# Gumo-A/hnsw_rs

Hardware: AMD Instinct MI355X
Metric: queries/sec at recall@10>=0.99, 1M x 100d L2 (higher is better)
Workload: dtype f32

## Files before the change

hnsw_rs_amd/csrc/capi.cpp:

```cpp

#include <hip/hip_runtime.h>

#include <linux/futex.h>
#include <sys/resource.h>
#include <sys/syscall.h>
#include <unistd.h>

#include <algorithm>
#include <atomic>
#include <chrono>
#include <climits>
#include <condition_variable>
#include <cstdio>
#include <cstdlib>
#include <cstring>
#include <memory>
#include <mutex>
#include <new>
#include <string>
#include <thread>
#include <vector>

#include "deleted.h"
#include "device_build.h"
#include "device_index.h"
#include "hip_util.h"
#include "host_index.h"
#include "search_filtered.h"

using hx::DevBuf;
using hx::set_error;

struct SearchScratch {
    void *dev = nullptr, *pin = nullptr;
    size_t dev_cap = 0, pin_cap = 0;
    hipStream_t stream = nullptr;
    int device = -1;
    ~SearchScratch() {
        if (dev) (void)hipFree(dev);
        if (pin) (void)hipHostFree(pin);
        if (stream) (void)hipStreamDestroy(stream);
    }
};

struct SpinLock {
    std::atomic<uint32_t> v{0};
    void lock() {
        for (int spins = 0; spins < 128; spins++) {
            uint32_t exp = 0;
            if (v.load(std::memory_order_relaxed) == 0 && v.compare_exchange_weak(exp, 1, std::memory_order_acquire)) return;
#if defined(__x86_64__)
            __builtin_ia32_pause();
#endif
        }
        while (v.exchange(2, std::memory_order_acquire) != 0)
            (void)syscall(SYS_futex, reinterpret_cast<uint32_t *>(&v), FUTEX_WAIT_PRIVATE, 2, nullptr, nullptr, 0);
    }
    void unlock() {
        if (v.exchange(0, std::memory_order_release) == 2)
            (void)syscall(SYS_futex, reinterpret_cast<uint32_t *>(&v), FUTEX_WAKE_PRIVATE, 1, nullptr, nullptr, 0);
    }
};

struct CoBatch {
    SearchScratch s;
    size_t p_q = 0, p_out = 0;
    std::atomic<uint32_t> cap{0}, n{0}, ef{0}, dim{0};
    static constexpr uint64_t COUNT = 0xFFFFull, CLOSED = 1ull << 16, GEN = 1ull << 32;
    std::atomic<uint64_t> word{CLOSED};
    std::atomic<uint32_t> filed{0};
    struct Req {
        uint32_t *ids, *count;
    };
    std::vector<Req> reqs;
    struct alignas(64) Word {
        std::atomic<uint32_t> v{0};
    };
    static constexpr uint32_t WORDS = 16;
    Word done[WORDS];
    std::atomic<uint32_t> readers{0};
    int rc = HNSW_OK;
    std::string err;
    std::vector<int32_t> status;
};
struct Coalescer {
    std::atomic<CoBatch *> fast{nullptr};
    SpinLock mu;
    std::condition_variable_any cv;
    std::vector<CoBatch *> open;
    std::vector<std::unique_ptr<CoBatch>> all;
    std::vector<CoBatch *> idle;
    uint32_t in_flight = 0;
    std::atomic<uint32_t> last_size{1};
    std::atomic<int64_t> window_us{30};
    uint32_t depth = 3, cap = 1024;
    std::atomic<uint64_t> n_batches{0}, n_queries{0}, max_batch{0};
    std::atomic<uint64_t> ns_window{0}, ns_turn{0}, ns_gpu{0}, ns_handout{0};
};

struct hnsw_index {
    std::unique_ptr<hx::HostIndex> host;
    hx::DeviceIndex dev;
    int device = -1;
    int gpu_build = 0;
    uint32_t build_batch_max = 8192, build_batch_div = 8;
    bool incomplete_build = false;
    bool cosine = false;
    std::mutex mu;
    std::mutex pool_mu;
    std::vector<std::unique_ptr<SearchScratch>> pool;
    Coalescer co;
    std::atomic<uint64_t> n_uploads{0}, n_point_patches{0}, n_patch_fallbacks{0};
    int64_t filter_exact_max = 65536;
    std::atomic<uint64_t> n_filt_graph{0}, n_filt_exact{0}, n_filt_overflow{0};
    hx::DeletedSet del;
    std::atomic<uint64_t> n_del_graph{0}, n_del_exact{0}, n_del_overflow{0};
    hx::BuildStats build;
};

namespace {

hx::BuildTarget build_target(hnsw_index *h) {
    return {*h->host, h->dev, h->device, {h->build_batch_max, h->build_batch_div}, h->build};
}

inline bool is_replica(const hnsw_index *h) { return h->dev.replica; }
inline uint64_t index_len(const hnsw_index *h) { return is_replica(h) ? h->dev.view.n_points : h->host->len(); }
int reject_replica(const hnsw_index *h, const char *what) {
    if (!is_replica(h)) return HNSW_OK;
    set_error("%s: this handle is a device-only replica (hnsw_snapshot_adopt); it holds no host copy of the index", what);
    return HNSW_ERR_ARG;
}

int cosine_rows(const hnsw_index *h, const float *&rows, uint64_t n, std::vector<float> &keep, uint32_t nb_threads = 1) {
    if (!h->cosine || !rows) return HNSW_OK;
    const uint32_t d = h->host->dim;
    keep.resize((size_t)n * d);
    std::atomic<uint64_t> bad{UINT64_MAX};
    auto work = [&](uint64_t lo, uint64_t hi) {
        for (uint64_t i = lo; i < hi; i++) {
            const float *x = rows + i * d;
            float s = 0.0f;
            for (uint32_t e = 0; e < d; e++) {
                const float t = x[e] * x[e];
                s += t;
            }
            const float nrm = sqrtf(s);
            if (!(nrm > 0.0f) || !std::isfinite(nrm)) {
                uint64_t cur = bad.load();
                while (i < cur && !bad.compare_exchange_weak(cur, i)) {
                }
                return;
            }
            float *y = &keep[(size_t)i * d];
            for (uint32_t e = 0; e < d; e++) y[e] = x[e] / nrm;
        }
    };
    const unsigned nt = (unsigned)std::min<uint64_t>(std::max(1u, nb_threads), std::max<uint64_t>(1, n / 4096));
    if (nt <= 1) {
        work(0, n);
    } else {
        std::vector<std::thread> th;
        for (unsigned t = 0; t < nt; t++) th.emplace_back(work, n * t / nt, n * (t + 1) / nt);
        for (auto &t : th) t.join();
    }
    if (bad.load() != UINT64_MAX) {
        set_error("row %llu has no direction (zero, NaN, or a norm outside f32's range): the cosine metric cannot place it",
                  (unsigned long long)bad.load());
        return HNSW_ERR_NAN_INPUT;
    }
    rows = keep.data();
    return HNSW_OK;
}
int cosine_queries(const hnsw_index *h, void *d_Q, uint64_t nq, hipStream_t stream) {
    if (!h->cosine) return HNSW_OK;
    return hx::launch_normalise_rows(static_cast<float *>(d_Q), nq, h->dev.view.dim, stream);
}

struct DeviceQueries {
    const float *q = nullptr;
    void *tmp = nullptr;
    hipStream_t st = nullptr;
    int prepare(const hnsw_index *h, const float *d_Q, uint64_t nq, hipStream_t stream) {
        q = d_Q;
        st = stream;
        if (!h->cosine) return HNSW_OK;
        const size_t bytes = (size_t)nq * h->dev.view.dim * 4;
        HIP_TRY(hipMallocAsync(&tmp, bytes, stream));
        HIP_TRY(hipMemcpyAsync(tmp, d_Q, bytes, hipMemcpyDeviceToDevice, stream));
        q = static_cast<const float *>(tmp);
        return hx::launch_normalise_rows(static_cast<float *>(tmp), nq, h->dev.view.dim, stream);
    }
    ~DeviceQueries() {
        if (tmp) (void)hipFreeAsync(tmp, st);
    }
};

int ensure_uploaded(hnsw_index *h) {
    std::lock_guard<std::mutex> g(h->mu);
    if (is_replica(h) && !h->dev.valid) {
        set_error("replica snapshot not committed (hnsw_snapshot_commit)");
        return HNSW_ERR_ARG;
    }
    if (!h->dev.current(*h->host)) {
        int rc = h->dev.upload(*h->host, h->device);
        if (rc != HNSW_OK) return rc;
        h->device = h->dev.device;
        h->n_uploads.fetch_add(1, std::memory_order_relaxed);
        hipMemPool_t pool = nullptr;
        if (hipDeviceGetDefaultMemPool(&pool, h->dev.device) == hipSuccess && pool != nullptr) {
            uint64_t keep = 1ull << 30;
            (void)hipMemPoolSetAttribute(pool, hipMemPoolAttrReleaseThreshold, &keep);
        }
        (void)hipGetLastError();
    }
    hipError_t e = hipSetDevice(h->dev.device);
    if (e != hipSuccess) {
        set_error("hipSetDevice(%d): %s", h->dev.device, hipGetErrorString(e));
        return HNSW_ERR_HIP;
    }
    return HNSW_OK;
}

int check_search_args(const hnsw_index *h, uint32_t ef) {
    if (!h) {
        set_error("null handle");
        return HNSW_ERR_ARG;
    }
    if (h->incomplete_build) {
        set_error("an on-device build on this handle failed half way; the index is incomplete, discard it");
        return HNSW_ERR_ARG;
    }
    if (index_len(h) == 0) {
        set_error("index is empty");
        return HNSW_ERR_EMPTY;
    }
    if (ef > (1u << 26)) {
        set_error("ef = %u is above 2^26", ef);
        return HNSW_ERR_ARG;
    }
    return HNSW_OK;
}

hx::SearchArgs ann_args(const hx::DevView &v, const float *dQ, uint32_t n, uint32_t ef,
                        uint32_t *ids, float *dists, uint32_t *counts, hnsw_query_stats *stats) {
    hx::SearchArgs a{};
    a.Q = dQ;
    a.qsel = nullptr;
    a.entries = nullptr;
    a.n_entry = 1;
    a.layer_hi = (int32_t)v.nb_layers - 1;
    a.layer_lo = 0;
    a.ef_upper = 1;
    a.ef_bottom = ef;
    a.n = n;
    a.out_ids = ids;
    a.out_dists = dists;
    a.out_counts = counts;
    a.out_stats = stats;
    return a;
}

struct ScratchLease {
    hnsw_index *h;
    std::unique_ptr<SearchScratch> s;
    explicit ScratchLease(hnsw_index *hh) : h(hh) {
        std::lock_guard<std::mutex> g(h->pool_mu);
        if (!h->pool.empty()) {
            s = std::move(h->pool.back());
            h->pool.pop_back();
        }
    }
    ~ScratchLease() {
        if (!s) return;
        std::lock_guard<std::mutex> g(h->pool_mu);
        if (h->pool.size() < 16) h->pool.push_back(std::move(s));
    }
    int prepare(int device, size_t dev_bytes, size_t pin_bytes) {
        if (s && s->device != device) s.reset();
        if (!s) {
            s.reset(new SearchScratch());
            s->device = device;
            HIP_TRY(hipStreamCreateWithFlags(&s->stream, hipStreamNonBlocking));
        }
        if (s->dev_cap < dev_bytes) {
            if (s->dev) (void)hipFree(s->dev);
            s->dev = nullptr;
            s->dev_cap = 0;
            const size_t cap = dev_bytes + dev_bytes / 4 + 4096;
            HIP_TRY(hipMalloc(&s->dev, cap));
            s->dev_cap = cap;
        }
        if (s->pin_cap < pin_bytes) {
            if (s->pin) (void)hipHostFree(s->pin);
            s->pin = nullptr;
            s->pin_cap = 0;
            const size_t cap = pin_bytes + pin_bytes / 4 + 4096;
            HIP_TRY(hipHostMalloc(&s->pin, cap, hipHostMallocDefault));
            s->pin_cap = cap;
        }
        return HNSW_OK;
    }
};

inline size_t align256(size_t x) { return (x + 255) & ~(size_t)255; }

struct HostSearchPlan {
    size_t o_q, o_sel, o_ent, o_out, dev_bytes;
    size_t r_ids, r_dists, r_counts, r_stats, out_bytes;
    size_t p_q, p_out, pin_bytes;
};
HostSearchPlan plan_host_search(uint64_t nq, uint32_t d, uint32_t n, uint32_t n_entry) {
    HostSearchPlan p{};
    p.o_q = 0;
    p.o_sel = p.o_q + align256(nq * d * 4);
    p.o_ent = p.o_sel + align256(nq * 4);
    p.o_out = p.o_ent + align256((size_t)n_entry * 4);
    p.r_ids = 0;
    p.r_dists = p.r_ids + align256(nq * n * 4);
    p.r_counts = p.r_dists + align256(nq * n * 4);
    p.r_stats = p.r_counts + align256(nq * 4);
    p.out_bytes = p.r_stats + align256(nq * sizeof(hnsw_query_stats));
    p.dev_bytes = p.o_out + p.out_bytes;
    p.p_q = 0;
    p.p_out = align256(nq * d * 4);
    p.pin_bytes = p.p_out + p.out_bytes;
    return p;
}

int query_status_error(uint64_t i, int32_t status) {
    switch (status) {
        case HNSW_OK:
            break;
        case HNSW_ERR_NAN_INPUT:
            set_error("query %llu: NaN in the query or in a distance", (unsigned long long)i);
            break;
        case HNSW_ERR_NODE_NOT_IN_GRAPH:
            set_error("Error in search_layer: node not in Graph (query %llu)", (unsigned long long)i);
            break;
        case HNSW_ERR_OVERFLOW:
            set_error("query %llu: visited table exhausted at its largest size", (unsigned long long)i);
            break;
        default:
            set_error("query %llu failed with status %d", (unsigned long long)i, status);
    }
    return status;
}

int search_staged(hnsw_index *h, SearchScratch &s, const HostSearchPlan &p, hx::SearchArgs a_host, uint64_t nq,
                  const uint32_t *entries, const float *Q_user) {
    const hx::DevView &v = h->dev.view;
    unsigned char *dv = static_cast<unsigned char *>(s.dev), *hv = static_cast<unsigned char *>(s.pin);
    int rc;
    static const bool zc_allowed = !(getenv("HNSW_MI355X_ZERO_COPY") && atoi(getenv("HNSW_MI355X_ZERO_COPY")) == 0);
    static const uint64_t zc_max = getenv("HNSW_MI355X_ZERO_COPY_MAX") ? strtoull(getenv("HNSW_MI355X_ZERO_COPY_MAX"), nullptr, 0) : 512;
    const bool zc = zc_allowed && !Q_user && !h->cosine && nq <= zc_max;
    hx::SearchArgs a = a_host;
    unsigned char *ob = zc ? hv + p.p_out : dv + p.o_out;
    if (zc) {
        a.Q = reinterpret_cast<const float *>(hv + p.p_q);
    } else {
        HIP_TRY(hipMemcpyAsync(dv + p.o_q, Q_user ? (const void *)Q_user : (const void *)(hv + p.p_q), nq * v.dim * 4,
                               hipMemcpyHostToDevice, s.stream));
        if ((rc = cosine_queries(h, dv + p.o_q, nq, s.stream))) return rc;
        a.Q = reinterpret_cast<const float *>(dv + p.o_q);
    }
    a.out_ids = reinterpret_cast<uint32_t *>(ob + p.r_ids);
    a.out_dists = reinterpret_cast<float *>(ob + p.r_dists);
    a.out_counts = reinterpret_cast<uint32_t *>(ob + p.r_counts);
    a.out_stats = reinterpret_cast<hnsw_query_stats *>(ob + p.r_stats);
    if (entries) {
        HIP_TRY(hipMemcpyAsync(dv + p.o_ent, entries, (size_t)a.n_entry * 4, hipMemcpyHostToDevice, s.stream));
        a.entries = reinterpret_cast<const uint32_t *>(dv + p.o_ent);
    }
    const hnsw_query_stats *st = reinterpret_cast<const hnsw_query_stats *>(hv + p.p_out + p.r_stats);
    uint32_t ef_max = std::max(a.ef_bottom, a.ef_upper);
    uint32_t slots = hx::default_slots_log2(ef_max, v.S0);
    uint64_t nrun = nq;
    std::vector<uint32_t> sel;
    while (true) {
        rc = hx::launch_search(v, a, (uint32_t)nrun, slots, s.stream);
        if (rc != HNSW_OK) return rc;
        if (!zc) HIP_TRY(hipMemcpyAsync(hv + p.p_out, dv + p.o_out, p.out_bytes, hipMemcpyDeviceToHost, s.stream));
        HIP_TRY(hipStreamSynchronize(s.stream));
        sel.clear();
        for (uint64_t i = 0; i < nq; i++)
            if (st[i].status == HNSW_ERR_OVERFLOW) sel.push_back((uint32_t)i);
        if (sel.empty() || slots >= hx::max_slots_log2(ef_max)) break;
        slots++;
        HIP_TRY(hipMemcpyAsync(dv + p.o_sel, sel.data(), sel.size() * 4, hipMemcpyHostToDevice, s.stream));
        HIP_TRY(hipStreamSynchronize(s.stream));
        a.qsel = reinterpret_cast<const uint32_t *>(dv + p.o_sel);
        nrun = sel.size();
    }
    return HNSW_OK;
}

int search_host(hnsw_index *h, hx::SearchArgs a_host, const float *Q, uint64_t nq, uint32_t *ids,
                float *dists, uint32_t *counts, hnsw_query_stats *stats, const uint32_t *entries) {
    int rc = ensure_uploaded(h);
    if (rc != HNSW_OK) return rc;
    const hx::DevView &v = h->dev.view;
    const uint32_t n = a_host.n, d = v.dim;
    const HostSearchPlan p = plan_host_search(nq, d, n, entries ? a_host.n_entry : 0);
    const bool stage_q = nq * (size_t)d * 4 <= (8u << 20);
    ScratchLease lease(h);
    if ((rc = lease.prepare(h->dev.device, p.dev_bytes, stage_q ? p.pin_bytes : p.out_bytes))) return rc;
    SearchScratch &s = *lease.s;
    HostSearchPlan pp = p;
    if (!stage_q) pp.p_out = 0;
    unsigned char *hv = static_cast<unsigned char *>(s.pin);
    if (stage_q) memcpy(hv + pp.p_q, Q, nq * (size_t)d * 4);
    if ((rc = search_staged(h, s, pp, a_host, nq, entries, stage_q ? nullptr : Q))) return rc;
    const unsigned char *ob = hv + pp.p_out;
    const hnsw_query_stats *st = reinterpret_cast<const hnsw_query_stats *>(ob + pp.r_stats);
    memcpy(ids, ob + pp.r_ids, nq * n * 4);
    if (dists) memcpy(dists, ob + pp.r_dists, nq * n * 4);
    if (counts) memcpy(counts, ob + pp.r_counts, nq * 4);
    if (stats) memcpy(stats, st, nq * sizeof(hnsw_query_stats));
    for (uint64_t i = 0; i < nq; i++)
        if (st[i].status != HNSW_OK) return query_status_error(i, st[i].status);
    return HNSW_OK;
}


struct PathCounters {
    std::atomic<uint64_t> *graph, *exact, *overflow;
};
const uint64_t kNoWords = 0;

PathCounters filt_counters(hnsw_index *h) { return {&h->n_filt_graph, &h->n_filt_exact, &h->n_filt_overflow}; }
PathCounters del_counters(hnsw_index *h) { return {&h->n_del_graph, &h->n_del_exact, &h->n_del_overflow}; }

int sync_deleted(hnsw_index *h) {
    if (h->del.count == 0) return HNSW_OK;
    std::lock_guard<std::mutex> g(h->mu);
    if (h->del.d_words && h->del.d_device == h->dev.device && h->del.dirty.empty()) return HNSW_OK;
    ScratchLease lease(h);
    int rc = lease.prepare(h->dev.device, 0, 0);
    if (rc != HNSW_OK) return rc;
    return h->del.sync(h->dev.device, lease.s->stream);
}

uint64_t count_admissible(const hnsw_index *h, const uint64_t *allow, uint64_t bits, std::vector<uint32_t> &wbase) {
    const uint64_t n_words = (bits + 63) / 64, n_wblk = (n_words + 63) / 64;
    const std::vector<uint64_t> &deny = h->del.words;
    const bool denies = h->del.count > 0;
    wbase.assign(std::max<uint64_t>(1, n_wblk), 0);
    uint64_t A = 0;
    for (uint64_t w = 0; w < n_words; w++) {
        if (w % 64 == 0) wbase[w / 64] = (uint32_t)A;
        uint64_t x = allow ? allow[w] : ~0ull;
        if (w == n_words - 1 && bits % 64) x &= (1ull << (bits % 64)) - 1;
        if (denies && w < deny.size()) x &= ~deny[w];
        A += (uint64_t)__builtin_popcountll(x);
    }
    return A;
}

int filtered_exact(const hx::DevView &v, const hx::FilterArgs &a, uint64_t nsel, const uint32_t *d_sel, uint64_t n_words,
                   const uint32_t *d_wb, uint32_t *d_ids, uint64_t A, uint32_t chunk, uint32_t nseg, void *part,
                   void *pst, hipStream_t stream) {
    int r = hx::launch_filter_compact(a, n_words, d_wb, d_ids, stream);
    for (uint64_t c = 0; r == HNSW_OK && c < nsel; c += chunk) {
        hx::FilterArgs ac = a;
        if (d_sel) {
            ac.qsel = d_sel + c;
        } else {
            ac.qsel = nullptr;
            ac.Q += c * v.dim;
            ac.out_ids += c * a.n;
            ac.out_dists += c * a.n;
            ac.out_counts += c;
            ac.out_stats += c;
        }
        r = hx::launch_filtered_exact(v, ac, (uint32_t)std::min<uint64_t>(chunk, nsel - c), d_ids, (uint32_t)A, nseg,
                                      static_cast<unsigned long long *>(part), static_cast<int32_t *>(pst), stream);
    }
    return r;
}

int search_filtered(hnsw_index *h, const float *Q, uint64_t nq, uint32_t n, uint32_t ef, const uint64_t *allow,
                    uint64_t allow_bits, bool exact_only, uint32_t *ids, float *dists, uint32_t *counts,
                    hnsw_query_stats *stats, uint8_t *paths, const PathCounters *ctr) {
    int rc = check_search_args(h, ef);
    if (rc != HNSW_OK) return rc;
    if (nq == 0) return HNSW_OK;
    if (!Q || !ids || nq > 0x7FFFFFFFull || n > HX_FILT_MAX_N) {
        set_error("filtered search: needs queries, an id buffer, a mask when allow_bits > 0 and n <= %d",
                  HX_FILT_MAX_N);
        return HNSW_ERR_ARG;
    }
    if (n == 0) {
        if (counts) memset(counts, 0, nq * 4);
        return HNSW_OK;
    }
    const uint32_t efp = std::max(std::max(ef, n), 1u);
    const uint64_t bits = std::min<uint64_t>(allow_bits, index_len(h));
    const uint64_t n_words = (bits + 63) / 64;
    std::vector<uint32_t> wbase;
    const uint64_t A = count_admissible(h, allow, bits, wbase);
    const bool exact_all = exact_only || (int64_t)A <= h->filter_exact_max;
    if (!exact_all && efp > HX_FILT_MAX_EF) {
        set_error("filtered search: ef' = max(ef, n) = %u is above the graph path's maximum of %d", efp, HX_FILT_MAX_EF);
        return HNSW_ERR_ARG;
    }
    if ((rc = ensure_uploaded(h)) || (rc = sync_deleted(h))) return rc;
    const hx::DevView &v = h->dev.view;
    const uint32_t d = v.dim;
    const uint32_t chunk = (uint32_t)std::min<uint64_t>(nq, 65535);
    const uint32_t nseg = hx::filt_exact_segments(A, chunk);
    const size_t o_q = 0, o_mask = o_q + align256(nq * d * 4), o_wb = o_mask + align256(allow ? n_words * 8 : 0),
                 o_ids = o_wb + align256(wbase.size() * 4), o_sel = o_ids + align256(A * 4),
                 o_part = o_sel + align256(nq * 4), o_pst = o_part + align256((size_t)chunk * nseg * n * 8),
                 o_out = o_pst + align256((size_t)chunk * nseg * 4);
    const size_t r_ids = 0, r_dists = align256(nq * n * 4), r_counts = r_dists + align256(nq * n * 4),
                 r_stats = r_counts + align256(nq * 4), out_bytes = r_stats + align256(nq * sizeof(hnsw_query_stats));
    ScratchLease lease(h);
    if ((rc = lease.prepare(h->dev.device, o_out + out_bytes, out_bytes))) return rc;
    SearchScratch &s = *lease.s;
    unsigned char *dv = static_cast<unsigned char *>(s.dev), *hv = static_cast<unsigned char *>(s.pin);
    HIP_TRY(hipMemcpyAsync(dv + o_q, Q, nq * d * 4, hipMemcpyHostToDevice, s.stream));
    if ((rc = cosine_queries(h, dv + o_q, nq, s.stream))) return rc;
    if (n_words) {
        if (allow) HIP_TRY(hipMemcpyAsync(dv + o_mask, allow, n_words * 8, hipMemcpyHostToDevice, s.stream));
        HIP_TRY(hipMemcpyAsync(dv + o_wb, wbase.data(), wbase.size() * 4, hipMemcpyHostToDevice, s.stream));
    }
    hx::FilterArgs a{};
    a.Q = reinterpret_cast<const float *>(dv + o_q);
    a.allow = allow ? reinterpret_cast<const uint64_t *>(dv + o_mask) : nullptr;
    a.allow_bits = bits;
    a.deny = h->del.count ? h->del.d_words : nullptr;
    a.deny_bits = h->del.count ? h->del.deny_bits() : 0;
    a.n = n;
    a.ef = efp;
    a.out_ids = reinterpret_cast<uint32_t *>(dv + o_out + r_ids);
    a.out_dists = reinterpret_cast<float *>(dv + o_out + r_dists);
    a.out_counts = reinterpret_cast<uint32_t *>(dv + o_out + r_counts);
    a.out_stats = reinterpret_cast<hnsw_query_stats *>(dv + o_out + r_stats);
    uint32_t *d_sel = reinterpret_cast<uint32_t *>(dv + o_sel);
    auto exact = [&](uint64_t nsel, bool selected) -> int {
        return filtered_exact(v, a, nsel, selected ? d_sel : nullptr, n_words,
                              reinterpret_cast<const uint32_t *>(dv + o_wb), reinterpret_cast<uint32_t *>(dv + o_ids), A,
                              chunk, nseg, dv + o_part, dv + o_pst, s.stream);
    };
    const hnsw_query_stats *st = reinterpret_cast<const hnsw_query_stats *>(hv + r_stats);
    std::vector<uint8_t> path(nq, exact_all ? 1 : 0);
    if (exact_all) {
        if ((rc = exact(nq, false))) return rc;
        HIP_TRY(hipMemcpyAsync(hv, dv + o_out, out_bytes, hipMemcpyDeviceToHost, s.stream));
        HIP_TRY(hipStreamSynchronize(s.stream));
    } else {
        uint32_t slots = hx::filt_first_slots_log2(v, efp);
        const uint32_t max_slots = hx::filt_max_slots_log2(v);
        uint64_t nrun = nq;
        std::vector<uint32_t> sel;
        while (true) {
            if ((rc = hx::launch_filtered_graph(v, a, (uint32_t)nrun, slots, s.stream))) return rc;
            HIP_TRY(hipMemcpyAsync(hv, dv + o_out, out_bytes, hipMemcpyDeviceToHost, s.stream));
            HIP_TRY(hipStreamSynchronize(s.stream));
            sel.clear();
            for (uint64_t i = 0; i < nq; i++)
                if (st[i].status == HNSW_ERR_OVERFLOW) sel.push_back((uint32_t)i);
            if (sel.empty()) break;
            HIP_TRY(hipMemcpyAsync(d_sel, sel.data(), sel.size() * 4, hipMemcpyHostToDevice, s.stream));
            if (slots >= max_slots) {
                for (uint32_t i : sel) path[i] = 2;
                if ((rc = exact(sel.size(), true))) return rc;
                HIP_TRY(hipMemcpyAsync(hv, dv + o_out, out_bytes, hipMemcpyDeviceToHost, s.stream));
                HIP_TRY(hipStreamSynchronize(s.stream));
                break;
            }
            HIP_TRY(hipStreamSynchronize(s.stream));
            slots++;
            a.qsel = d_sel;
            nrun = sel.size();
        }
    }
    uint64_t n2 = 0;
    for (uint64_t i = 0; i < nq; i++) n2 += path[i] == 2;
    if (ctr) {
        if (exact_all)
            ctr->exact->fetch_add(nq, std::memory_order_relaxed);
        else
            ctr->graph->fetch_add(nq - n2, std::memory_order_relaxed);
        ctr->overflow->fetch_add(n2, std::memory_order_relaxed);
    }
    memcpy(ids, hv + r_ids, nq * n * 4);
    if (dists) memcpy(dists, hv + r_dists, nq * n * 4);
    if (counts) memcpy(counts, hv + r_counts, nq * 4);
    memcpy(stats, st, nq * sizeof(hnsw_query_stats));
    if (paths) memcpy(paths, path.data(), nq);
    return HNSW_OK;
}

int search_filtered_checked(hnsw_index *h, const float *Q, uint64_t nq, uint32_t n, uint32_t ef, const uint64_t *allow,
                            uint64_t allow_bits, bool exact_only, uint32_t *ids, float *dists, uint32_t *counts,
                            hnsw_query_stats *stats, uint8_t *paths, const PathCounters *ctr) {
    std::vector<hnsw_query_stats> local;
    if (!stats) {
        local.resize(nq);
        stats = local.data();
    }
    int rc = search_filtered(h, Q, nq, n, ef, allow, allow_bits, exact_only, ids, dists, counts, stats, paths, ctr);
    if (rc != HNSW_OK || n == 0) return rc;
    for (uint64_t i = 0; i < nq; i++)
        if (stats[i].status != HNSW_OK) return query_status_error(i, stats[i].status);
    return HNSW_OK;
}

int search_device_deleted(hnsw_index *h, const float *d_Q, uint64_t nq, uint32_t n, uint32_t ef, uint32_t *d_ids,
                          float *d_dists, uint32_t *d_counts, hnsw_query_stats *d_stats, hipStream_t stream, bool finish) {
    const uint32_t efp = std::max(std::max(ef, n), 1u);
    if (n > HX_FILT_MAX_N || efp > HX_FILT_MAX_EF) {
        set_error("search with deleted ids: needs n <= %d and ef' = max(ef, n) <= %d", HX_FILT_MAX_N, HX_FILT_MAX_EF);
        return HNSW_ERR_ARG;
    }
    int rc;
    if ((rc = ensure_uploaded(h)) || (rc = sync_deleted(h))) return rc;
    const hx::DevView &v = h->dev.view;
    DeviceQueries dq;
    if ((rc = dq.prepare(h, d_Q, nq, stream))) return rc;
    struct Tmp {
        void *p = nullptr;
        hipStream_t st = nullptr;
        ~Tmp() {
            if (p) (void)hipFreeAsync(p, st);
        }
    } t_dists, t_counts;
    if (!d_dists) {
        HIP_TRY(hipMallocAsync(&t_dists.p, nq * n * 4, stream));
        t_dists.st = stream;
        d_dists = static_cast<float *>(t_dists.p);
    }
    if (!d_counts) {
        HIP_TRY(hipMallocAsync(&t_counts.p, nq * 4, stream));
        t_counts.st = stream;
        d_counts = static_cast<uint32_t *>(t_counts.p);
    }
    hx::FilterArgs a{};
    a.Q = dq.q;
    a.allow = nullptr;
    a.allow_bits = index_len(h);
    a.deny = h->del.d_words;
    a.deny_bits = h->del.deny_bits();
    a.n = n;
    a.ef = efp;
    a.out_ids = d_ids;
    a.out_dists = d_dists;
    a.out_counts = d_counts;
    a.out_stats = d_stats;
    uint32_t slots = hx::filt_first_slots_log2(v, efp);
    if (!finish) return hx::launch_filtered_graph(v, a, (uint32_t)nq, slots, stream);

    const uint32_t max_slots = hx::filt_max_slots_log2(v);
    const size_t st_bytes = nq * sizeof(hnsw_query_stats);
    ScratchLease lease(h);
    if ((rc = lease.prepare(h->dev.device, align256(nq * 4), st_bytes))) return rc;
    hnsw_query_stats *st = static_cast<hnsw_query_stats *>(lease.s->pin);
    uint32_t *d_sel = static_cast<uint32_t *>(lease.s->dev);
    std::vector<uint32_t> sel;
    uint64_t n2 = 0;
    while (true) {
        HIP_TRY(hipMemcpyAsync(st, d_stats, st_bytes, hipMemcpyDeviceToHost, stream));
        HIP_TRY(hipStreamSynchronize(stream));
        sel.clear();
        for (uint64_t i = 0; i < nq; i++)
            if (st[i].status == HNSW_ERR_OVERFLOW) sel.push_back((uint32_t)i);
        if (sel.empty()) break;
        if (slots >= max_slots) {
            n2 = sel.size();
            std::vector<uint32_t> wbase;
            const uint64_t bits = a.allow_bits, n_words = (bits + 63) / 64;
            const uint64_t A = count_admissible(h, nullptr, bits, wbase);
            const uint32_t chunk = (uint32_t)std::min<uint64_t>(n2, 65535);
            const uint32_t nseg = hx::filt_exact_segments(A, chunk);
            const size_t o_sel = 0, o_wb = align256(n2 * 4), o_ids = o_wb + align256(wbase.size() * 4),
                         o_part = o_ids + align256(A * 4), o_pst = o_part + align256((size_t)chunk * nseg * n * 8),
                         bytes = o_pst + align256((size_t)chunk * nseg * 4);
            if ((rc = lease.prepare(h->dev.device, bytes, st_bytes))) return rc;
            unsigned char *dv = static_cast<unsigned char *>(lease.s->dev);
            st = static_cast<hnsw_query_stats *>(lease.s->pin);
            HIP_TRY(hipMemcpyAsync(dv + o_sel, sel.data(), n2 * 4, hipMemcpyHostToDevice, stream));
            HIP_TRY(hipMemcpyAsync(dv + o_wb, wbase.data(), wbase.size() * 4, hipMemcpyHostToDevice, stream));
            if ((rc = filtered_exact(v, a, n2, reinterpret_cast<const uint32_t *>(dv + o_sel), n_words,
                                     reinterpret_cast<const uint32_t *>(dv + o_wb), reinterpret_cast<uint32_t *>(dv + o_ids),
// ... 1376 lines not shown
```

Before: 6.065 million.

## Write search outputs directly to pinned host memory and pre-create pool streams

Search results (ids, dists, counts, stats) are now always written by the kernel straight into pinned host memory, even on the non-zero-copy path. This removes the device output buffer and the device-to-host copy after each launch. The first lease also creates several scratch streams up front so later concurrent searches do not pay stream creation cost. In exchange, large batches now write their outputs over the host interconnect, which may be slower than device writes followed by one bulk copy.

After: 6.044 million (median of 2 runs). About the same (-0.4%).

```diff
diff --git a/hnsw_rs_amd/csrc/capi.cpp b/hnsw_rs_amd/csrc/capi.cpp
--- a/hnsw_rs_amd/csrc/capi.cpp
+++ b/hnsw_rs_amd/csrc/capi.cpp
@@ -109,6 +109,7 @@
     std::mutex mu;
     std::mutex pool_mu;
     std::vector<std::unique_ptr<SearchScratch>> pool;
+    bool pool_primed = false;
     Coalescer co;
     std::atomic<uint64_t> n_uploads{0}, n_point_patches{0}, n_patch_fallbacks{0};
     int64_t filter_exact_max = 65536;
@@ -261,14 +262,19 @@
     return a;
 }
 
+constexpr unsigned kPoolStreamsUpFront = 4;
+
 struct ScratchLease {
     hnsw_index *h;
     std::unique_ptr<SearchScratch> s;
+    bool first = false;
     explicit ScratchLease(hnsw_index *hh) : h(hh) {
         std::lock_guard<std::mutex> g(h->pool_mu);
         if (!h->pool.empty()) {
             s = std::move(h->pool.back());
             h->pool.pop_back();
+        } else if (!h->pool_primed) {
+            h->pool_primed = first = true;
         }
     }
     ~ScratchLease() {
@@ -276,12 +282,24 @@
         std::lock_guard<std::mutex> g(h->pool_mu);
         if (h->pool.size() < 16) h->pool.push_back(std::move(s));
     }
+    static int make(int device, std::unique_ptr<SearchScratch> &out) {
+        out.reset(new SearchScratch());
+        out->device = device;
+        HIP_TRY(hipStreamCreateWithFlags(&out->stream, hipStreamNonBlocking));
+        HIP_TRY(hipStreamSynchronize(out->stream));
+        return HNSW_OK;
+    }
     int prepare(int device, size_t dev_bytes, size_t pin_bytes) {
         if (s && s->device != device) s.reset();
         if (!s) {
-            s.reset(new SearchScratch());
-            s->device = device;
-            HIP_TRY(hipStreamCreateWithFlags(&s->stream, hipStreamNonBlocking));
+            int rc = make(device, s);
+            if (rc != HNSW_OK) return rc;
+            for (unsigned i = 1; first && i < kPoolStreamsUpFront; i++) {
+                std::unique_ptr<SearchScratch> more;
+                if ((rc = make(device, more))) return rc;
+                std::lock_guard<std::mutex> g(h->pool_mu);
+                h->pool.insert(h->pool.begin(), std::move(more));
+            }
         }
         if (s->dev_cap < dev_bytes) {
             if (s->dev) (void)hipFree(s->dev);
@@ -306,7 +324,7 @@
 inline size_t align256(size_t x) { return (x + 255) & ~(size_t)255; }
 
 struct HostSearchPlan {
-    size_t o_q, o_sel, o_ent, o_out, dev_bytes;
+    size_t o_q, o_sel, o_ent, dev_bytes;
     size_t r_ids, r_dists, r_counts, r_stats, out_bytes;
     size_t p_q, p_out, pin_bytes;
 };
@@ -315,13 +333,12 @@
     p.o_q = 0;
     p.o_sel = p.o_q + align256(nq * d * 4);
     p.o_ent = p.o_sel + align256(nq * 4);
-    p.o_out = p.o_ent + align256((size_t)n_entry * 4);
     p.r_ids = 0;
     p.r_dists = p.r_ids + align256(nq * n * 4);
     p.r_counts = p.r_dists + align256(nq * n * 4);
     p.r_stats = p.r_counts + align256(nq * 4);
     p.out_bytes = p.r_stats + align256(nq * sizeof(hnsw_query_stats));
-    p.dev_bytes = p.o_out + p.out_bytes;
+    p.dev_bytes = p.o_ent + align256((size_t)n_entry * 4);
     p.p_q = 0;
     p.p_out = align256(nq * d * 4);
     p.pin_bytes = p.p_out + p.out_bytes;
@@ -356,7 +373,7 @@
     static const uint64_t zc_max = getenv("HNSW_MI355X_ZERO_COPY_MAX") ? strtoull(getenv("HNSW_MI355X_ZERO_COPY_MAX"), nullptr, 0) : 512;
     const bool zc = zc_allowed && !Q_user && !h->cosine && nq <= zc_max;
     hx::SearchArgs a = a_host;
-    unsigned char *ob = zc ? hv + p.p_out : dv + p.o_out;
+    unsigned char *ob = hv + p.p_out;
     if (zc) {
         a.Q = reinterpret_cast<const float *>(hv + p.p_q);
     } else {
@@ -381,7 +398,6 @@
     while (true) {
         rc = hx::launch_search(v, a, (uint32_t)nrun, slots, s.stream);
         if (rc != HNSW_OK) return rc;
-        if (!zc) HIP_TRY(hipMemcpyAsync(hv + p.p_out, dv + p.o_out, p.out_bytes, hipMemcpyDeviceToHost, s.stream));
         HIP_TRY(hipStreamSynchronize(s.stream));
         sel.clear();
         for (uint64_t i = 0; i < nq; i++)
```
